# microsoft/EVA

Hardware: AMD Instinct MI355X
Metric: homomorphic ops/sec (mul+rescale+relin) at N=2^16, L=10; execute() wall-time (higher is better)
Workload: dtype u64

## Files before the change

eva_amd/csrc/internal.hip.h:

```cpp
#pragma once
#include "../../include/eva_hip.h"

#include <hip/hip_runtime.h>

#include <algorithm>
#include <cmath>
#include <cstdlib>
#include <cstring>
#include <functional>
#include <map>
#include <memory>
#include <mutex>
#include <stdexcept>
#include <string>
#include <tuple>
#include <unordered_map>
#include <vector>

#include "devmath.hip.h"
#include "hostmath.h"

namespace evah {

extern thread_local std::string g_err;

void ctx_register(const void *c);
void ctx_unregister(const void *c);
bool ctx_alive(const void *c);

#define HIPCHK(x)                                                                                \
  do {                                                                                           \
    hipError_t e_ = (x);                                                                         \
    if (e_ != hipSuccess)                                                                        \
      throw std::runtime_error(std::string(#x) + " failed: " + hipGetErrorString(e_));          \
  } while (0)

#ifndef EVAH_KS_BATCH_MAX_DEFINED
#define EVAH_KS_BATCH_MAX_DEFINED
constexpr int KS_BATCH_MAX = 64;
#endif


struct Pool {
  std::map<size_t, std::vector<void *>> free_;
  size_t in_use = 0, cached = 0;
  void *alloc(size_t bytes) {
    bytes = (bytes + 255) & ~(size_t)255;
    auto it = free_.find(bytes);
    void *p = nullptr;
    if (it != free_.end() && !it->second.empty()) {
      p = it->second.back();
      it->second.pop_back();
      cached -= bytes;
    } else {
      hipError_t e = hipMalloc(&p, bytes);
      if (e != hipSuccess) {
        release_cached();
        HIPCHK(hipMalloc(&p, bytes));
      }
    }
    in_use += bytes;
    return p;
  }
  void free(void *p, size_t bytes) {
    bytes = (bytes + 255) & ~(size_t)255;
    free_[bytes].push_back(p);
    in_use -= bytes;
    cached += bytes;
  }
  void release_cached() {
    for (auto &kv : free_)
      for (void *p : kv.second) (void)hipFree(p);
    free_.clear();
    cached = 0;
  }
};

struct Buffer {
  u64 *d;
  size_t bytes;
  int refs;
  Pool *pool;
  evah_ctx *owner;
  bool ready_everywhere;
  std::vector<evah_ctx *> synced;
  std::vector<evah_ctx *> readers;
};

enum KClass {
  KC_EW = 0,
  KC_INTT_A,
  KC_INTT_B,
  KC_KSDIGIT_A,
  KC_KSDIGIT_B,
  KC_KSMAC,
  KC_MODDOWN_A,
  KC_MODDOWN_B,
  KC_NTT_A,
  KC_NTT_B,
  KC_COUNT
};
static const char *const kclass_names[KC_COUNT] = {
    "elementwise", "intt_pass1", "intt_pass2", "ksdigit_pass1", "ksdigit_pass2", "ks_mac",
    "moddown_pass1", "moddown_pass2", "ntt_pass1", "ntt_pass2"};

struct ProfRec {
  hipEvent_t e0, e1;
  int cls;
};

__host__ __device__ inline size_t keyp_block_words(uint32_t nd) { return ((size_t)2 * nd + 1) * 256; }
struct KeyDev {
  u64 *d = nullptr;
  uint32_t n_digits = 0;
  size_t bytes = 0;
  uint32_t rows = 0;
  u64 *d_split = nullptr;
  u64 *d_perm = nullptr;
};

}

using namespace evah;

struct evah_ct {
  Buffer *buf;
  u64 *d;
  uint32_t size, limbs;
  size_t ps;
  double scale;
  uint32_t batch = 1;
};
struct evah_pt {
  Buffer *buf;
  u64 *d;
  uint32_t limbs;
  double scale;
  bool uniform = false;
};
struct evah_graph {
  hipGraph_t graph = nullptr;
  hipGraphExec_t exec = nullptr;
  struct Reserved { evah_ctx *ctx; void *p; size_t bytes; };
  std::vector<Reserved> reserved;
};

struct SharedDev {
  int device = 0;
  void *d_tables = nullptr;
  KeyDev relin;
  KeyDev pk, sk;
  double2 *dec_roots = nullptr;
  std::map<uint32_t, u64 *> crt_tabs;
  std::map<uint32_t, KeyDev> galois;
  std::map<uint32_t, uint32_t *> perms;
  std::map<uint32_t, uint32_t *> perms_inv;
  std::map<uint32_t, u64 *> hoist_sign;
  std::map<std::pair<uint32_t, uint32_t>, u64 *> hoist_corr;
  double2 *enc_roots = nullptr;
  double enc_last_root[2] = {0, 0};
  uint32_t *enc_slot_map = nullptr;
  uint32_t key_rows = 0, key_shard = 0;
  uint64_t xfer[6] = {0, 0, 0, 0, 0, 0};
  uint64_t key_up[2] = {0, 0};
  ~SharedDev() {
    (void)hipSetDevice(device);
    if (enc_roots) (void)hipFree(enc_roots);
    if (enc_slot_map) (void)hipFree(enc_slot_map);
    if (relin.d) (void)hipFree(relin.d);
    if (relin.d_split) (void)hipFree(relin.d_split);
    if (pk.d) (void)hipFree(pk.d);
    if (sk.d) { (void)hipMemset(sk.d, 0, sk.bytes); (void)hipFree(sk.d); }
    if (dec_roots) (void)hipFree(dec_roots);
    for (auto &kv : crt_tabs) (void)hipFree(kv.second);
    for (auto &kv : galois) {
      (void)hipFree(kv.second.d);
      if (kv.second.d_split) (void)hipFree(kv.second.d_split);
      if (kv.second.d_perm) (void)hipFree(kv.second.d_perm);
    }
    for (auto &kv : perms) (void)hipFree(kv.second);
    for (auto &kv : perms_inv) (void)hipFree(kv.second);
    for (auto &kv : hoist_sign) (void)hipFree(kv.second);
    for (auto &kv : hoist_corr) (void)hipFree(kv.second);
    if (d_tables) (void)hipFree(d_tables);
  }
};

struct Tunables {
  bool fuse_mac = true;
  bool fuse_mul = true;
  bool fuse_mul2 = true;
  bool ew_fuse = true;
  bool ew_uniform = true;
  uint32_t fuse_small_blocks = 2048;
  int small_lr = 2;
  uint32_t small_lr_blocks = 1024;
  bool hoist = true;
  uint32_t hoist_min_tiles = 2048;
  bool hoist_debug = false;
  bool peer_self_check = false;
  bool hoist_table_fail = false;
  bool fuse_special_inv = true;
  int ks_groups = 1;
  int ks_threads = 64;
  bool fold_pa = true;
  bool win_fuse = true;
  bool win_linear = true;
  bool fb_persist = true;
  uint32_t fb_grid = 0;
  bool mac3 = true;
  uint32_t loop_n = 8, loop_min = 2, loop_min_wgs = 2048, loop_target_wgs = 8192;
  bool hoist_map = true;
  uint32_t hoist_v = 1;
  bool side_stream = false;
  bool chain_step = true, chain_batched = true;
  uint32_t chain_fuse_blocks = 256;
  bool modup = true;
  uint32_t lds_extra = 0;

  static Tunables from_env(uint32_t N) {
    Tunables t;
    auto flag = [](const char *name, bool &v) { if (const char *e = std::getenv(name)) v = std::atoi(e) != 0; };
    auto count = [](const char *name, uint32_t &v) { if (const char *e = std::getenv(name)) v = (uint32_t)std::max(0, std::atoi(e)); };
    (void)N;
    flag("EVAH_FUSE_MAC", t.fuse_mac);
    flag("EVAH_FUSE_MUL", t.fuse_mul);
    flag("EVAH_FUSE_MUL2", t.fuse_mul2);
    flag("EVAH_EW_FUSE", t.ew_fuse);
    flag("EVAH_EW_UNIFORM", t.ew_uniform);
    count("EVAH_FUSE_SMALL", t.fuse_small_blocks);
    if (const char *e = std::getenv("EVAH_SMALL_LR")) t.small_lr = std::atoi(e) == 3 ? 3 : 2;
    count("EVAH_SMALL_LR_BLOCKS", t.small_lr_blocks);
    flag("EVAH_HOIST", t.hoist);
    count("EVAH_HOIST_MIN_TILES", t.hoist_min_tiles);
    flag("EVAH_HOIST_DEBUG", t.hoist_debug);
    flag("EVAH_HOIST_TABLE_FAIL", t.hoist_table_fail);
    flag("EVAH_PEER_SELF_CHECK", t.peer_self_check);
    flag("EVAH_FUSE_SPECIAL_INV", t.fuse_special_inv);
    flag("EVAH_FOLD_PA", t.fold_pa);
    flag("EVAH_WIN_FUSE", t.win_fuse);
    flag("EVAH_WIN_LINEAR", t.win_linear);
    flag("EVAH_FB_PERSIST", t.fb_persist);
    count("EVAH_FB_GRID", t.fb_grid);
    flag("EVAH_MAC3", t.mac3);
    count("EVAH_LOOP_N", t.loop_n);
    count("EVAH_LOOP_MIN", t.loop_min);
    count("EVAH_LOOP_MIN_WGS", t.loop_min_wgs);
    count("EVAH_LOOP_TARGET_WGS", t.loop_target_wgs);
    count("EVAH_LDS_EXTRA", t.lds_extra);
    flag("EVAH_HOIST_MAP", t.hoist_map);
    flag("EVAH_SIDE_STREAM", t.side_stream);
    flag("EVAH_CHAIN_STEP", t.chain_step);
    flag("EVAH_CHAIN_BATCHED", t.chain_batched);
    count("EVAH_CHAIN_FUSE_BLOCKS", t.chain_fuse_blocks);
    flag("EVAH_MODUP", t.modup);
    count("EVAH_HOIST_V", t.hoist_v);
    if (const char *e = std::getenv("EVAH_KS_GROUPS")) t.ks_groups = std::max(1, std::atoi(e));
    if (const char *e = std::getenv("EVAH_KS_THREADS")) {
      const int n = std::atoi(e);
      if (n == 64 || n == 128 || n == 256) t.ks_threads = n;
    }
    return t;
  }
};

struct evah_ctx {
  std::shared_ptr<SharedDev> sh;
  int device = 0;
  uint32_t N = 0, logN = 0, k = 0;
  std::vector<u64> primes;
  std::vector<int> total_bits;
  DevCtx dev{};
  hipStream_t own = nullptr, stream = nullptr;
  hipStream_t side = nullptr;
  Pool pool;
  hipEvent_t ev0 = nullptr, ev1 = nullptr;
  bool capturing = false;
  std::vector<hipEvent_t> capture_events;
  std::vector<hipEvent_t> sync_events;
  Tunables tun;
  bool all_tb = false;
  bool prof_on = false;
  std::vector<ProfRec> prof_recs;
  std::vector<hipEvent_t> prof_free;
  double prof_ms[KC_COUNT] = {0};
  uint64_t prof_n[KC_COUNT] = {0};
};

namespace evah {

inline void use(evah_ctx *c) { HIPCHK(hipSetDevice(c->device)); }
inline void count_h2d(evah_ctx *c, size_t bytes, bool plain = false) { c->sh->xfer[plain ? 2 : 0]++; c->sh->xfer[4] += bytes; }
inline void count_d2h(evah_ctx *c, size_t bytes, bool plain = false) { c->sh->xfer[plain ? 3 : 1]++; c->sh->xfer[5] += bytes; }

inline hipEvent_t prof_event(evah_ctx *c) {
  if (!c->prof_free.empty()) {
    hipEvent_t e = c->prof_free.back();
    c->prof_free.pop_back();
    return e;
  }
  hipEvent_t e;
  HIPCHK(hipEventCreate(&e));
  return e;
}
inline void prof_drain(evah_ctx *c) {
  for (auto &r : c->prof_recs) {
    float ms = 0;
    HIPCHK(hipEventSynchronize(r.e1));
    HIPCHK(hipEventElapsedTime(&ms, r.e0, r.e1));
    c->prof_ms[r.cls] += ms;
    c->prof_n[r.cls]++;
    c->prof_free.push_back(r.e0);
    c->prof_free.push_back(r.e1);
  }
  c->prof_recs.clear();
}
struct ProfScope {
  evah_ctx *c;
  int cls;
  hipEvent_t e0 = nullptr;
  ProfScope(evah_ctx *c_, int cls_) : c(c_), cls(cls_) {
    if (c->prof_on && !c->capturing) {
      if (c->prof_recs.size() >= 8192) prof_drain(c);
      e0 = prof_event(c);
      HIPCHK(hipEventRecord(e0, c->stream));
    }
  }
  ~ProfScope() {
    if (e0) {
      hipEvent_t e1 = prof_event(c);
      (void)hipEventRecord(e1, c->stream);
      c->prof_recs.push_back({e0, e1, cls});
    }
  }
};

inline Buffer *buf_new(evah_ctx *c, size_t elems) {
  Buffer *b = new Buffer;
  b->bytes = elems * sizeof(u64);
  b->d = (u64 *)c->pool.alloc(b->bytes);
  b->refs = 1;
  b->pool = &c->pool;
  b->owner = c;
  b->ready_everywhere = false;
  return b;
}
inline void h2d_now(evah_ctx *c, void *dst, const void *src, size_t bytes) {
  HIPCHK(hipMemcpyAsync(dst, src, bytes, hipMemcpyHostToDevice, c->stream));
  HIPCHK(hipStreamSynchronize(c->stream));
}
inline hipEvent_t sync_event(evah_ctx *c) {
  if (!c->capturing && !c->sync_events.empty()) {
    hipEvent_t e = c->sync_events.back();
    c->sync_events.pop_back();
    return e;
  }
  hipEvent_t e;
  HIPCHK(hipEventCreateWithFlags(&e, hipEventDisableTiming));
  return e;
}
inline void stream_wait(evah_ctx *waiter, evah_ctx *signaller) {
  if (waiter == signaller || waiter->stream == signaller->stream) return;
  if (waiter->sh.get() != signaller->sh.get()) {
    int cur = 0;
    HIPCHK(hipGetDevice(&cur));
    HIPCHK(hipSetDevice(signaller->device));
    hipEvent_t e = sync_event(signaller);
    hipError_t rc = hipEventRecord(e, signaller->stream);
    (void)hipSetDevice(waiter->device);
    if (rc == hipSuccess) rc = hipStreamWaitEvent(waiter->stream, e, 0);
    (void)hipSetDevice(cur);
    if (waiter->capturing || signaller->capturing) signaller->capture_events.push_back(e);
    else signaller->sync_events.push_back(e);
    HIPCHK(rc);
    return;
  }
  hipEvent_t e = sync_event(waiter);
  HIPCHK(hipEventRecord(e, signaller->stream));
  HIPCHK(hipStreamWaitEvent(waiter->stream, e, 0));
  if (waiter->capturing || signaller->capturing) waiter->capture_events.push_back(e);
  else waiter->sync_events.push_back(e);
}
struct SideStream {
  evah_ctx *c;
  hipStream_t main;
  bool forked = false, on_side = false;
  explicit SideStream(evah_ctx *c_) : c(c_), main(c_->stream) {}
  void link(hipStream_t from, hipStream_t to) {
    hipEvent_t e = sync_event(c);
    HIPCHK(hipEventRecord(e, from));
    HIPCHK(hipStreamWaitEvent(to, e, 0));
    if (c->capturing) c->capture_events.push_back(e);
    else c->sync_events.push_back(e);
  }
  void fork() {
    if (!c->side) HIPCHK(hipStreamCreateWithFlags(&c->side, hipStreamNonBlocking));
    link(main, c->side);
    c->stream = c->side;
    forked = on_side = true;
  }
  void back() { c->stream = main; on_side = false; }
  void join() {
    back();
    if (forked) link(c->side, main);
    forked = false;
  }
  ~SideStream() {
    c->stream = main;
    if (forked) {
      hipEvent_t e = sync_event(c);
      if (hipEventRecord(e, c->side) == hipSuccess) (void)hipStreamWaitEvent(main, e, 0);
      (c->capturing ? c->capture_events : c->sync_events).push_back(e);
    }
  }
};
inline void acquire(evah_ctx *c, Buffer *b) {
  if (!b || b->owner == c) return;
  if (!b->ready_everywhere && std::find(b->synced.begin(), b->synced.end(), c) == b->synced.end()) {
    stream_wait(c, b->owner);
    b->synced.push_back(c);
  }
  if (std::find(b->readers.begin(), b->readers.end(), c) == b->readers.end()) b->readers.push_back(c);
}
inline void buf_unref(evah_ctx *c, Buffer *b) {
  (void)c;
  if (b && --b->refs == 0) {
    if (!ctx_alive(b->owner)) {
      (void)hipFree(b->d);
      delete b;
      return;
    }
    for (evah_ctx *r : b->readers)
      if (ctx_alive(r)) stream_wait(b->owner, r);
    b->pool->free(b->d, b->bytes);
    delete b;
  }
}
inline evah_ct *ct_new(evah_ctx *c, uint32_t size, uint32_t limbs, double scale, uint32_t batch = 1) {
  evah_ct *t = new evah_ct;
  t->batch = batch;
  t->buf = buf_new(c, (size_t)batch * size * limbs * c->N);
  t->d = t->buf->d;
  t->size = size;
  t->limbs = limbs;
  t->ps = (size_t)limbs * c->N;
  t->scale = scale;
  return t;
}
inline evah_pt *pt_new(evah_ctx *c, uint32_t limbs, double scale) {
  evah_pt *t = new evah_pt;
  t->buf = buf_new(c, (size_t)limbs * c->N);
  t->d = t->buf->d;
  t->limbs = limbs;
  t->scale = scale;
  return t;
}

bool hoist_wanted(const evah_ctx *c, uint32_t l, uint32_t n, uint32_t B);

KeyDev key_shape(evah_ctx *c, uint32_t n_digits);
hipError_t key_rows_h2d(evah_ctx *c, const KeyDev &kd, const u64 *src, uint32_t blocks, uint32_t first, uint32_t step);
void key_install(evah_ctx *c, int kind, uint32_t galois_elt, const KeyDev &kd);

struct Scratch {
  evah_ctx *c;
  u64 *d;
  size_t bytes;
  Scratch(evah_ctx *c_, size_t elems) : c(c_), bytes(elems * sizeof(u64)) {
    d = (u64 *)c->pool.alloc(bytes);
  }
  ~Scratch() { c->pool.free(d, bytes); }
};

inline dim3 ew_grid(evah_ctx *c, uint32_t limbs, uint32_t polys) {
  return dim3(c->N / 512, limbs, polys);
}

inline int bitlen_of_product(const std::vector<u64> &primes, uint32_t count) {
  std::vector<u64> w{1};
  for (uint32_t i = 0; i < count; i++) {
    u64 carry = 0;
    for (auto &x : w) {
      u128 t = (u128)x * primes[i] + carry;
      x = (u64)t;
      carry = (u64)(t >> 64);
    }
    if (carry) w.push_back(carry);
  }
  int bits = (int)(w.size() - 1) * 64;
  u64 top = w.back();
  while (top) { bits++; top >>= 1; }
  return bits;
}

inline void check_scale(evah_ctx *c, double scale, uint32_t limbs) {
  if (!(scale > 0) || (int)std::log2(scale) >= c->total_bits[limbs])
    throw std::invalid_argument("scale out of bounds");
}
inline bool same_scale(double a, double b) {
  double scale_factor = std::max({std::fabs(a), std::fabs(b), 1.0});
  return std::fabs(a - b) < 2.220446049250313e-16 * scale_factor;
}

}

#define EW_LAUNCH(...) do { ProfScope ps_(c, KC_EW); hipLaunchKernelGGL(__VA_ARGS__); } while (0)
#define API_BEGIN try {
#define API_END                                                                                  \
  g_err.clear();                                                                                 \
  return 0;                                                                                      \
  }                                                                                              \
  catch (const std::exception &e) {                                                              \
    g_err = e.what();                                                                            \
    return 1;                                                                                    \
  }                                                                                              \
  catch (...) {                                                                                  \
    g_err = "unknown error";                                                                     \
    return 1;                                                                                    \
  }
```

eva_amd/csrc/launch.hip.h:

```cpp
#pragma once
#include "internal.hip.h"
#include "ntt.hip.h"

namespace evah {

#define EW_SETUP                                                                                 \
  const uint32_t p = blockIdx.z, i = blockIdx.y;                                                 \
  const size_t off = (size_t)i * cx.N + 2 * ((size_t)blockIdx.x * blockDim.x + threadIdx.x);    \
  const DevPrime pm = cx.primes[cx.prime_of(i)];                                                 \
  (void)p;                                                                                        \
  (void)pm;

__device__ __forceinline__ ulonglong2 ld2(const u64 *p) { return *reinterpret_cast<const ulonglong2 *>(p); }
__device__ __forceinline__ void st2(u64 *p, ulonglong2 v) { *reinterpret_cast<ulonglong2 *>(p) = v; }
__device__ __forceinline__ u64 split30(u64 k) { return (k & 0x3fffffffull) | ((k >> 30) << 32); }

template <class Op> struct OpClass;
template <bool Z, bool G> struct OpClass<OpPlainT<Z, G>> { static constexpr int fwd_a = KC_NTT_A, fwd_b = KC_NTT_B; };
template <> struct OpClass<OpMulIntt> { static constexpr int fwd_a = KC_NTT_A, fwd_b = KC_NTT_B; };
template <> struct OpClass<OpKsDigit> { static constexpr int fwd_a = KC_KSDIGIT_A, fwd_b = KC_KSDIGIT_B; };
template <bool G> struct OpClass<OpModDownT<G>> { static constexpr int fwd_a = KC_MODDOWN_A, fwd_b = KC_MODDOWN_B; };
template <> struct OpClass<OpMulPolyIntt> { static constexpr int fwd_a = KC_NTT_A, fwd_b = KC_NTT_B; };
template <> struct OpClass<OpModDownMul> { static constexpr int fwd_a = KC_MODDOWN_A, fwd_b = KC_MODDOWN_B; };
template <int M> struct OpClass<OpRRT<M>> { static constexpr int fwd_a = KC_MODDOWN_A, fwd_b = KC_MODDOWN_B; };
template <int M> struct OpClass<OpRRLastT<M>> { static constexpr int fwd_a = KC_MODDOWN_A, fwd_b = KC_MODDOWN_B; };
template <> struct OpClass<OpChainIntt> { static constexpr int fwd_a = KC_NTT_A, fwd_b = KC_NTT_B; };
template <> struct OpClass<OpChainT> { static constexpr int fwd_a = KC_INTT_B, fwd_b = KC_INTT_B; };
template <> struct OpClass<OpChainDigit> { static constexpr int fwd_a = KC_KSDIGIT_A, fwd_b = KC_KSDIGIT_B; };
template <> struct OpClass<OpRsMd> { static constexpr int fwd_a = KC_MODDOWN_A, fwd_b = KC_MODDOWN_B; };

template <int P, int LR, bool STRIDED, bool INVERSE, class Op>
static void launch_pass(evah_ctx *c, const typename Op::Params &prm, uint32_t jobs) {
  ProfScope ps(c, INVERSE ? (STRIDED ? KC_INTT_B : KC_INTT_A)
                          : (STRIDED ? OpClass<Op>::fwd_a : OpClass<Op>::fwd_b));
  const uint32_t max_tile = (uint32_t)NTT_THREADS << LR;
  const uint32_t tile = c->N < max_tile ? c->N : max_tile;
  const int logC = (int)ilog2(tile) - P;
  size_t lds = ((((size_t)1 << logC) * lds_sub_stride<P>() + 1) & ~(size_t)1) * sizeof(u64);
  if (STRIDED) lds += ((size_t)1 << P) * sizeof(ulonglong2);
  lds += c->tun.lds_extra;
  const uint32_t n_tiles = c->N / tile;
  const int log_tiles = (int)ilog2(n_tiles);
  dim3 grid = Op::grid(prm, jobs), block(tile >> LR);
  grid.x *= n_tiles;
  if (tile == max_tile) {
    hipLaunchKernelGGL((ntt_pass_kernel<P, LR, STRIDED, INVERSE, Op, true>), grid, block, lds, c->stream, c->dev,
                       prm, logC, log_tiles);
  } else if constexpr (P == 5) {
    hipLaunchKernelGGL((ntt_pass_kernel<P, LR, STRIDED, INVERSE, Op, false>), grid, block, lds, c->stream, c->dev,
                       prm, logC, log_tiles);
  } else {
    throw std::logic_error("partial NTT tile with P != 5");
  }
  HIPCHK(hipGetLastError());
}

template <int LR, bool STRIDED, bool INVERSE, class Op>
static void launch_pass_lr(evah_ctx *c, int P, const typename Op::Params &prm, uint32_t jobs) {
  switch (P) {
  case 5: launch_pass<5, LR, STRIDED, INVERSE, Op>(c, prm, jobs); break;
  case 6: launch_pass<6, LR, STRIDED, INVERSE, Op>(c, prm, jobs); break;
  case 7: launch_pass<7, LR, STRIDED, INVERSE, Op>(c, prm, jobs); break;
  case 8: launch_pass<8, LR, STRIDED, INVERSE, Op>(c, prm, jobs); break;
  case 9:
    if constexpr (STRIDED) { launch_pass<9, LR, STRIDED, INVERSE, Op>(c, prm, jobs); break; }
    [[fallthrough]];
  default: throw std::runtime_error("unsupported poly_modulus_degree for the NTT kernels");
  }
}
template <int P, bool INVERSE, class Op>
static bool launch_loop_pass(evah_ctx *c, const typename Op::Params &prm, uint32_t jobs) {
  constexpr int LR = 2;
  dim3 grid = Op::grid(prm, jobs);
  uint32_t ext[3] = {grid.x, grid.y, grid.z};
  const uint32_t count = ext[Op::loop_axis];
  if (!c->tun.loop_n || count < c->tun.loop_min || c->N < 256) return false;
  if ((uint64_t)ext[0] * ext[1] * ext[2] / count * (c->N / 256) * ((count + 1) / 2) < c->tun.loop_min_wgs) return false;
  ProfScope ps(c, INVERSE ? KC_INTT_A : OpClass<Op>::fwd_b);
  const uint32_t tile = 256, n_tiles = c->N / tile;
  const int logC = 8 - P, log_tiles = (int)ilog2(n_tiles);
  uint32_t nloop = std::min<uint32_t>(c->tun.loop_n, count);
  const uint64_t others = (uint64_t)ext[0] * ext[1] * ext[2] / count * n_tiles;
  while (nloop > 2 && others * ((count + nloop - 1) / nloop) < c->tun.loop_target_wgs) nloop = (nloop + 1) / 2;
  ext[Op::loop_axis] = (count + nloop - 1) / nloop;
  const size_t lds = ((((size_t)1 << logC) * lds_sub_stride<P>() + 1) & ~(size_t)1) * sizeof(u64) +
                     ((size_t)1 << (logC + P)) * sizeof(ulonglong2);
  hipLaunchKernelGGL((ntt_loop_kernel<P, LR, INVERSE, Op>), dim3(ext[0] * n_tiles, ext[1], ext[2]), dim3(tile >> LR), lds, c->stream,
                     c->dev, prm, logC, log_tiles, nloop, count);
  HIPCHK(hipGetLastError());
  return true;
}
template <bool INVERSE, class Op>
static bool launch_loop_pass_p(evah_ctx *c, int P, const typename Op::Params &prm, uint32_t jobs) {
  switch (P) {
  case 5: return launch_loop_pass<5, INVERSE, Op>(c, prm, jobs);
  case 6: return launch_loop_pass<6, INVERSE, Op>(c, prm, jobs);
  case 7: return launch_loop_pass<7, INVERSE, Op>(c, prm, jobs);
  case 8: return launch_loop_pass<8, INVERSE, Op>(c, prm, jobs);
  default: return false;
  }
}

template <bool STRIDED, bool INVERSE, class Op>
static void launch_pass_p(evah_ctx *c, int P, const typename Op::Params &prm, uint32_t jobs) {
  if constexpr (!STRIDED) {
    if (launch_loop_pass_p<INVERSE, Op>(c, P, prm, jobs)) return;
  }
  if (c->tun.small_lr == 2 && (uint64_t)jobs * (c->N >> 11) <= c->tun.small_lr_blocks && c->N >= 2048) {
    launch_pass_lr<2, STRIDED, INVERSE, Op>(c, P, prm, jobs);
    return;
  }
  launch_pass_lr<3, STRIDED, INVERSE, Op>(c, P, prm, jobs);
}

struct KsBatch {
  uint32_t n = 1;
  uint32_t i0 = 0, ni = 0;
  size_t target_bs = 0, scratch_bs = 0, prod_bs = 0;
  KsKeys keys{};
  PtrTab targets{};
  const MulTab *mul = nullptr;
  bool fold = false;
  const PtrTab *adds = nullptr;
  bool mac3 = false;
  bool lazy_out = false;
  uint32_t istep = 1, nout = 0;
  u64 *r_out = nullptr;
  bool diag = false;
  uint32_t fold_row = ~0u;
};
void launch_ks_inner(evah_ctx *c, int P, const u64 *target, const u64 *scratch, const KsBatch &key, u64 *prod, uint32_t l);

template <class Op> static void ntt_forward(evah_ctx *c, const typename Op::Params &prm, uint32_t jobs) {
  const int a = (c->logN + 1) / 2, b = c->logN / 2;
  launch_pass_p<true, false, Op>(c, a, prm, jobs);
  launch_pass_p<false, false, Op>(c, b, prm, jobs);
}
template <class Op> static void ntt_inverse(evah_ctx *c, const typename Op::Params &prm, uint32_t jobs) {
  const int a = (c->logN + 1) / 2, b = c->logN / 2;
  launch_pass_p<false, true, Op>(c, b, prm, jobs);
  launch_pass_p<true, true, Op>(c, a, prm, jobs);
}

static inline bool fuse_small_launch(evah_ctx *c, uint32_t fwd_jobs) {
  const uint32_t tile = (uint32_t)NTT_THREADS << 3;
  if (!c->tun.fuse_small_blocks || c->N < tile) return false;
  if (c->dev.guard) return true;
  return (uint64_t)fwd_jobs * (c->N / tile) <= c->tun.fuse_small_blocks;
}
template <int P, class Op, int LR> static void launch_inv_fwd_plr(evah_ctx *c, const typename Op::Params &prm, uint32_t jobs) {
  ProfScope ps(c, OpClass<Op>::fwd_a);
  const uint32_t tile = (uint32_t)NTT_THREADS << LR, n_tiles = c->N / tile;
  const int logC = (int)ilog2(tile) - P;
  const size_t lds = ((((size_t)1 << logC) * lds_sub_stride<P>() + 1) & ~(size_t)1) * sizeof(u64) + 2 * ((size_t)1 << P) * sizeof(ulonglong2);
  dim3 grid = Op::grid(prm, jobs);
  grid.x *= n_tiles;
  hipLaunchKernelGGL((ntt_inv_fwd_kernel<P, LR, Op>), grid, dim3(NTT_THREADS), lds, c->stream, c->dev, prm, (int)ilog2(n_tiles));
  HIPCHK(hipGetLastError());
}
template <int P, class Op> static void launch_inv_fwd_p(evah_ctx *c, const typename Op::Params &prm, uint32_t jobs) {
  if (c->tun.small_lr == 2) launch_inv_fwd_plr<P, Op, 2>(c, prm, jobs);
  else launch_inv_fwd_plr<P, Op, 3>(c, prm, jobs);
}
template <class Op> static void launch_inv_fwd(evah_ctx *c, const typename Op::Params &prm, uint32_t jobs) {
  switch ((c->logN + 1) / 2) {
  case 6: launch_inv_fwd_p<6, Op>(c, prm, jobs); break;
  case 7: launch_inv_fwd_p<7, Op>(c, prm, jobs); break;
  case 8: launch_inv_fwd_p<8, Op>(c, prm, jobs); break;
  case 9: launch_inv_fwd_p<9, Op>(c, prm, jobs); break;
  default: throw std::runtime_error("unsupported poly_modulus_degree for the fused inverse/forward pass");
  }
}
static inline bool modup_fits(evah_ctx *c) { return c->N >= ((uint32_t)NTT_THREADS << 3) && (c->logN + 1) / 2 <= 9; }
template <int P, class Op> static void launch_modup_p(evah_ctx *c, const typename Op::Params &prm, uint32_t n) {
  ProfScope ps(c, OpClass<Op>::fwd_a);
  constexpr int LR = 3;
  const uint32_t tile = (uint32_t)NTT_THREADS << LR, n_tiles = c->N / tile;
  const int logC = (int)ilog2(tile) - P;
  const size_t lds = ((((size_t)1 << logC) * lds_sub_stride<P>() + 1) & ~(size_t)1) * sizeof(u64) + ((size_t)1 << P) * sizeof(ulonglong2);
  hipLaunchKernelGGL((ntt_modup_kernel<P, LR, Op>), dim3(n_tiles * prm.l, 1, n), dim3(NTT_THREADS), lds, c->stream, c->dev, prm,
                     (int)ilog2(n_tiles));
  HIPCHK(hipGetLastError());
}
template <class Op> static void launch_modup(evah_ctx *c, const typename Op::Params &prm, uint32_t n) {
  if (!modup_fits(c) || prm.i0 != 0 || prm.istep != 1) throw std::logic_error("mod-up kernel outside its shapes");
  switch ((c->logN + 1) / 2) {
  case 6: launch_modup_p<6, Op>(c, prm, n); break;
  case 7: launch_modup_p<7, Op>(c, prm, n); break;
  case 8: launch_modup_p<8, Op>(c, prm, n); break;
  case 9: launch_modup_p<9, Op>(c, prm, n); break;
  default: throw std::runtime_error("unsupported poly_modulus_degree for the mod-up kernel");
  }
}
template <int P, class Op, bool FWD, int LR> static void launch_inv2_plr(evah_ctx *c, const typename Op::Params &prm, uint32_t jobs) {
  ProfScope ps(c, OpClass<Op>::fwd_a);
  const uint32_t tile = (uint32_t)NTT_THREADS << LR, n_tiles = c->N / tile;
  const int logC = (int)ilog2(tile) - P;
  const size_t lds = ((((size_t)1 << logC) * lds_sub_stride<P>() + 1) & ~(size_t)1) * sizeof(u64) + 2 * ((size_t)1 << P) * sizeof(ulonglong2);
  dim3 grid = Op::grid(prm, jobs);
  grid.x *= n_tiles;
  hipLaunchKernelGGL((ntt_inv2_kernel<P, LR, Op, FWD>), grid, dim3(NTT_THREADS), lds, c->stream, c->dev, prm, (int)ilog2(n_tiles));
  HIPCHK(hipGetLastError());
}
template <class Op, bool FWD> static void launch_inv2(evah_ctx *c, const typename Op::Params &prm, uint32_t jobs) {
  auto go = [&](auto ptag) {
    constexpr int P = decltype(ptag)::value;
    if (c->tun.small_lr == 2) launch_inv2_plr<P, Op, FWD, 2>(c, prm, jobs);
    else launch_inv2_plr<P, Op, FWD, 3>(c, prm, jobs);
  };
  switch ((c->logN + 1) / 2) {
  case 6: go(std::integral_constant<int, 6>{}); break;
  case 7: go(std::integral_constant<int, 7>{}); break;
  case 8: go(std::integral_constant<int, 8>{}); break;
  case 9: go(std::integral_constant<int, 9>{}); break;
  default: throw std::runtime_error("unsupported poly_modulus_degree for the fused inverse/forward pass");
  }
}
template <class InvOp, class Op>
static void inverse_then_forward(evah_ctx *c, const typename InvOp::Params &ip, uint32_t inv_jobs, const typename Op::Params &fp,
                                 uint32_t fwd_jobs, bool inv_pass1_done = false) {
  if (inv_pass1_done && !fuse_small_launch(c, fwd_jobs)) throw std::logic_error("fused inverse pass outside the small-launch form");
  if (fuse_small_launch(c, fwd_jobs)) {
    if (!inv_pass1_done) launch_pass_p<false, true, InvOp>(c, c->logN / 2, ip, inv_jobs);
    launch_inv_fwd<Op>(c, fp, fwd_jobs);
    launch_pass_p<false, false, Op>(c, c->logN / 2, fp, fwd_jobs);
  } else {
    ntt_inverse<InvOp>(c, ip, inv_jobs);
    ntt_forward<Op>(c, fp, fwd_jobs);
  }
}

bool switch_key_products(evah_ctx *c, uint32_t l, const u64 *target, size_t target_bs, const KeyDev *const *keys, uint32_t n,
                         u64 *prod_d, const PtrTab *target_tab = nullptr, const MulTab *mul = nullptr, u64 *r_small = nullptr,
                         bool fold = false, const PtrTab *adds = nullptr, bool lazy_out = false);
void switch_key(evah_ctx *c, uint32_t l, const u64 *target, const KeyDev &key, const u64 *add, size_t add_ps, uint32_t add_polys,
                u64 *out, size_t out_ps);
void key_split_launch(evah_ctx *c, const u64 *src, u64 *dst, size_t words);
const uint32_t *perm_table(evah_ctx *c, uint32_t elt);
void galois_perm_launch(evah_ctx *c, const u64 *a, size_t a_ps, uint32_t limbs, uint32_t polys, const uint32_t *perm, u64 *out, size_t o_ps);
void enc_tables(evah_ctx *c);

}
```

eva_amd/csrc/ntt_modup.hip.h:

```cpp
#pragma once
#include "ntt.hip.h"

namespace evah {

template <int P, int LR, class Op>
__global__ void __launch_bounds__(NTT_THREADS)
ntt_modup_kernel(DevCtx cx, typename Op::Params prm, int log_tiles) {
  extern __shared__ __attribute__((aligned(16))) u64 lds[];
  constexpr int NTT_R = 1 << LR;
  constexpr int S = 1 << P, TPS = S / NTT_R, SP = lds_sub_stride<P>();
  constexpr int logC = 8 + LR - P, C = 1 << logC, T = NTT_THREADS;
  constexpr int TWR = (S + T - 1) / T;
  if (cx.skipped()) return;
  const uint32_t tile_idx = blockIdx.x & ((1u << log_tiles) - 1u), J = blockIdx.x >> log_tiles, b = blockIdx.z;
  typename Op::Job jb;
  uint32_t iy = 0;
  while (iy < prm.ni && !Op::setup(cx, prm, J, iy, b, jb)) iy++;
  if (iy >= prm.ni) return;
  const uint32_t pa = Op::pre_prime(prm, jb);
  const DevPrime pmA = cx.primes[pa];
  const uint32_t stride_log = cx.logN - P;
  constexpr int ES = 1 << (P - LR);
  constexpr bool LINEAR = (ES % 16 == 0);
  const int c = threadIdx.x & (C - 1), e0 = threadIdx.x >> logC;
  const uint32_t n0 = (tile_idx << logC) + ((uint32_t)e0 << stride_log) + c, nstep = (uint32_t)(T >> logC) << stride_log;
  const int l0 = c * SP + lds_pad<P>(e0);
  auto lds_at = [&](int it) -> int {
    if constexpr (LINEAR) return l0 + it * lds_pad<P>(ES);
    const int idx = threadIdx.x + it * T;
    return (idx & (C - 1)) * SP + lds_pad<P>(idx >> logC);
  };
  const u64 *src = Op::pre_src(jb);
#pragma unroll
  for (int it = 0; it < NTT_R; it++) lds[lds_at(it)] = src[n0 + it * nstep];
  ulonglong2 *twl = reinterpret_cast<ulonglong2 *>(lds + ((C * SP + 1) & ~1));
  const ulonglong2 *twA = cx.tw_inv + (size_t)pa * cx.N;
  for (int idx = threadIdx.x; idx < S; idx += T) twl[idx] = twA[idx];
  ulonglong2 twn[TWR];
  auto tw_request = [&](uint32_t prime) {
    const ulonglong2 *tw = cx.tw_fwd + (size_t)prime * cx.N;
#pragma unroll
    for (int r = 0; r < TWR; r++)
      if (S >= T || (int)threadIdx.x + r * T < S) twn[r] = tw[threadIdx.x + r * T];
  };
  tw_request(jb.prime);
  __syncthreads();
  const int sub = threadIdx.x / TPS, tid = threadIdx.x % TPS;
  RoundSeq<P, LR, 0, true, true, false>::run(lds + sub * SP, tid, 0, 0, twl, pmA);
  __syncthreads();
  u64 t[NTT_R];
#pragma unroll
  for (int it = 0; it < NTT_R; it++) {
    t[it] = lds[lds_at(it)];
    if (Op::pre_addhalf) t[it] = addmod(t[it], pmA.q >> 1, pmA.q);
  }
  while (true) {
#pragma unroll
    for (int r = 0; r < TWR; r++)
      if (S >= T || (int)threadIdx.x + r * T < S) twl[threadIdx.x + r * T] = twn[r];
    const DevPrime pm = cx.primes[jb.prime];
    auto convert = [&](auto lazy_tag) {
      constexpr bool LZ = decltype(lazy_tag)::value;
#pragma unroll
      for (int it = 0; it < NTT_R; it++) lds[lds_at(it)] = Op::template conv<LZ>(jb, pm, t[it]);
    };
    if (jb.lazy) convert(std::true_type{});
    else convert(std::false_type{});
    typename Op::Job jn;
    uint32_t in = iy + 1;
    while (in < prm.ni && !Op::setup(cx, prm, J, in, b, jn)) in++;
    const bool more = in < prm.ni;
    if (more) tw_request(jn.prime);
    __syncthreads();
    forward_rounds<P, LR, true, false>(lds + sub * SP, tid, 0, 0, twl, pm);
    __syncthreads();
#pragma unroll
    for (int it = 0; it < NTT_R; it++) jb.dst[n0 + it * nstep] = lds[lds_at(it)];
    if (!more) break;
    jb = jn;
    iy = in;
  }
}

}
```

Before: 15590.

## Keep mod-up NTT data in registers across rounds with double-buffered twiddles

Adds a register-resident variant of the fused inverse-NTT/base-conversion/forward-NTT mod-up kernel. The inverse result stays in registers, and each output prime's conversion and first forward round start straight from registers instead of a full LDS write and read-back. It also uses a new column-padded LDS layout and double-buffers the forward twiddles so staging the next prime overlaps the current one. The variant is on by default behind a tunable; it needs more LDS for the second twiddle buffer and more registers, which may lower occupancy.

```diff
diff --git a/eva_amd/csrc/internal.hip.h b/eva_amd/csrc/internal.hip.h
--- a/eva_amd/csrc/internal.hip.h
+++ b/eva_amd/csrc/internal.hip.h
@@ -216,6 +216,7 @@
   bool chain_step = true, chain_batched = true;
   uint32_t chain_fuse_blocks = 256;
   bool modup = true;
+  bool modup_regs = true;
   uint32_t lds_extra = 0;
 
   static Tunables from_env(uint32_t N) {
@@ -254,6 +255,7 @@
     flag("EVAH_CHAIN_BATCHED", t.chain_batched);
     count("EVAH_CHAIN_FUSE_BLOCKS", t.chain_fuse_blocks);
     flag("EVAH_MODUP", t.modup);
+    flag("EVAH_MODUP_REGS", t.modup_regs);
     count("EVAH_HOIST_V", t.hoist_v);
     if (const char *e = std::getenv("EVAH_KS_GROUPS")) t.ks_groups = std::max(1, std::atoi(e));
     if (const char *e = std::getenv("EVAH_KS_THREADS")) {
diff --git a/eva_amd/csrc/launch.hip.h b/eva_amd/csrc/launch.hip.h
--- a/eva_amd/csrc/launch.hip.h
+++ b/eva_amd/csrc/launch.hip.h
@@ -176,10 +176,14 @@
   ProfScope ps(c, OpClass<Op>::fwd_a);
   constexpr int LR = 3;
   const uint32_t tile = (uint32_t)NTT_THREADS << LR, n_tiles = c->N / tile;
-  const int logC = (int)ilog2(tile) - P;
-  const size_t lds = ((((size_t)1 << logC) * lds_sub_stride<P>() + 1) & ~(size_t)1) * sizeof(u64) + ((size_t)1 << P) * sizeof(ulonglong2);
-  hipLaunchKernelGGL((ntt_modup_kernel<P, LR, Op>), dim3(n_tiles * prm.l, 1, n), dim3(NTT_THREADS), lds, c->stream, c->dev, prm,
-                     (int)ilog2(n_tiles));
+  const dim3 grid(n_tiles * prm.l, 1, n);
+  constexpr size_t lds_regs = modup_lds_bytes<P, LR, true>(), lds_tile = modup_lds_bytes<P, LR, false>();
+  if (c->tun.modup_regs)
+    hipLaunchKernelGGL((ntt_modup_kernel<P, LR, Op, true>), grid, dim3(NTT_THREADS), lds_regs, c->stream, c->dev, prm,
+                       (int)ilog2(n_tiles));
+  else
+    hipLaunchKernelGGL((ntt_modup_kernel<P, LR, Op, false>), grid, dim3(NTT_THREADS), lds_tile, c->stream, c->dev, prm,
+                       (int)ilog2(n_tiles));
   HIPCHK(hipGetLastError());
 }
 template <class Op> static void launch_modup(evah_ctx *c, const typename Op::Params &prm, uint32_t n) {
diff --git a/eva_amd/csrc/ntt_modup.hip.h b/eva_amd/csrc/ntt_modup.hip.h
--- a/eva_amd/csrc/ntt_modup.hip.h
+++ b/eva_amd/csrc/ntt_modup.hip.h
@@ -3,7 +3,202 @@
 
 namespace evah {
 
+template <int P> struct ModupTile {
+  static constexpr int SH = P == 6 ? 4 : P == 8 ? 2 : 3;
+  static constexpr int SP = P == 6 ? 69 : P == 7 ? 143 : P == 8 ? 322 : 580;
+  static __device__ __forceinline__ int pad(int e) { return e + (e >> SH); }
+  static_assert(SP >= (1 << P) + (((1 << P) - 1) >> SH), "a column holds every padded element");
+};
+template <int P, int LR, int RB, int LO> struct ColRound {
+  static constexpr int NTT_R = 1 << LR, TPS = (1 << P) >> LR, G = NTT_R >> RB, NU = 1 << RB;
+  static constexpr int S0 = P - LO - RB;
+  using L = ModupTile<P>;
+  static __device__ __forceinline__ int o_hi(int g, int p) { return (g * TPS + p) >> LO; }
+  static __device__ __forceinline__ int ebase(int g, int p) {
+    const int o = g * TPS + p;
+    return ((o >> LO) << (LO + RB)) | (o & ((1 << LO) - 1));
+  }
+  static __device__ __forceinline__ void load(const u64 *col, int p, u64 (&x)[NTT_R]) {
+#pragma unroll
+    for (int g = 0; g < G; g++) {
+      const u64 *grp = col + L::pad(ebase(g, p));
+#pragma unroll
+      for (int u = 0; u < NU; u++) x[g * NU + u] = grp[L::pad(u << LO)];
+    }
+  }
+  static __device__ __forceinline__ void store(u64 *col, int p, const u64 (&x)[NTT_R]) {
+#pragma unroll
+    for (int g = 0; g < G; g++) {
+      u64 *grp = col + L::pad(ebase(g, p));
+#pragma unroll
+      for (int u = 0; u < NU; u++) grp[L::pad(u << LO)] = x[g * NU + u];
+    }
+  }
+  template <bool TB> static __device__ __forceinline__ void fwd(int p, u64 (&x)[NTT_R], const ulonglong2 *tw, const DevPrime &pm) {
+    const u64 nq = pm.nq, q4 = pm.q4, q8 = pm.q8, nq8 = pm.nq8;
+    constexpr bool MAD = EVAH_MADLO && LR == 3;
+#pragma unroll
+    for (int g = 0; g < G; g++) {
+      const uint32_t node = (1u << S0) | (uint32_t)o_hi(g, p);
+#pragma unroll
+      for (int s = 0; s < RB; s++) {
+        const int half = 1 << (RB - 1 - s);
+#pragma unroll
+        for (int u = 0; u < NU; u++) {
+          if (u & half) continue;
+          const int v = u >> (RB - s);
+          const ulonglong2 w = tw[(node << s) + v];
+          const bool red = TB ? tb_reduce_stage<P, false>(S0 + s) : (((S0 + s) & 1) != 0);
+          if (red) bfly_fwd<true, MAD, TB>(x[g * NU + u], x[g * NU + u + half], w, nq, q4, q8, nq8, pm.tb_c, pm.tb_sh, pm.tb_mask);
+          else bfly_fwd<false, MAD, TB>(x[g * NU + u], x[g * NU + u + half], w, nq, q4, q8, nq8, pm.tb_c, pm.tb_sh, pm.tb_mask);
+        }
+      }
+    }
+  }
+  static __device__ __forceinline__ void inv(int p, u64 (&x)[NTT_R], const ulonglong2 *tw, const DevPrime &pm) {
+    const u64 q = pm.q, nq = pm.nq, q5 = pm.q5, nq5 = pm.nq5;
+#pragma unroll
+    for (int g = 0; g < G; g++) {
+      const uint32_t node = (1u << S0) | (uint32_t)o_hi(g, p);
+#pragma unroll
+      for (int s = RB - 1; s >= 0; s--) {
+        const int half = 1 << (RB - 1 - s);
+        const bool last = (S0 == 0) && (s == 0);
+#pragma unroll
+        for (int u = 0; u < NU; u++) {
+          if (u & half) continue;
+          u64 &X = x[g * NU + u], &Y = x[g * NU + u + half];
+          if (last) {
+            u64 sum = X + Y, d = X + q5 - Y;
+            X = mul_shoup(sum, pm.ninv, pm.ninv_s, q);
+            Y = mul_shoup(d, pm.w0ninv, pm.w0ninv_s, q);
+          } else {
+            const int v = u >> (RB - s);
+            bfly_inv(X, Y, tw[((size_t)node << s) + v], nq, q5, nq5);
+          }
+        }
+      }
+    }
+  }
+};
+template <int P, int LR, int I, bool TB> struct ColFwd {
+  using RS = Rounds<P, LR>;
+  using R = ColRound<P, LR, RS::bits(I), RS::lo(I)>;
+  static __device__ __forceinline__ void run(u64 *col, int p_in, u64 (&x)[1 << LR], const ulonglong2 *tw, const DevPrime &pm) {
+    int p = p_in;
+    if constexpr (I > 0) R::load(col, p, x);
+    else if constexpr (TB) asm volatile("" : "+v"(p));
+    R::template fwd<TB>(p, x, tw, pm);
+    if constexpr (I + 1 < RS::NR) {
+      R::store(col, p, x);
+      __syncthreads();
+      ColFwd<P, LR, I + 1, TB>::run(col, p, x, tw, pm);
+    }
+  }
+};
+template <int P, int LR, int I> struct ColInv {
+  using RS = Rounds<P, LR>;
+  static constexpr int idx = RS::NR - 1 - I;
+  using R = ColRound<P, LR, RS::bits(idx), RS::lo(idx)>;
+  static __device__ __forceinline__ void run(u64 *col, int p, u64 (&x)[1 << LR], const ulonglong2 *tw, const DevPrime &pm) {
+    R::load(col, p, x);
+    R::inv(p, x, tw, pm);
+    if constexpr (idx > 0) {
+      R::store(col, p, x);
+      __syncthreads();
+      ColInv<P, LR, I + 1>::run(col, p, x, tw, pm);
+    }
+  }
+};
+template <int P, int LR, bool REGS> constexpr size_t modup_lds_bytes() {
+  constexpr size_t C = (size_t)1 << (8 + LR - P), S = (size_t)1 << P;
+  if (REGS) return ((C * ModupTile<P>::SP + 1) & ~(size_t)1) * sizeof(u64) + 2 * S * sizeof(ulonglong2);
+  return ((C * lds_sub_stride<P>() + 1) & ~(size_t)1) * sizeof(u64) + S * sizeof(ulonglong2);
+}
+
 template <int P, int LR, class Op>
+__device__ __forceinline__ void modup_regs(const DevCtx &cx, const typename Op::Params &prm, int log_tiles, u64 *lds) {
+  constexpr int NTT_R = 1 << LR;
+  constexpr int S = 1 << P, TPS = S / NTT_R;
+  constexpr int logC = 8 + LR - P, C = 1 << logC, T = NTT_THREADS;
+  constexpr int TWR = (S + T - 1) / T;
+  using L = ModupTile<P>;
+  using RS = Rounds<P, LR>;
+  using RLast = ColRound<P, LR, RS::bits(RS::NR - 1), 0>;
+  static_assert(RS::bits(0) == LR && RS::lo(0) == P - LR && RS::lo(RS::NR - 1) == 0, "round 0 works on the load mapping's elements");
+  const uint32_t tile_idx = blockIdx.x & ((1u << log_tiles) - 1u), J = blockIdx.x >> log_tiles, b = blockIdx.z;
+  typename Op::Job jb;
+  uint32_t iy = 0;
+  while (iy < prm.ni && !Op::setup(cx, prm, J, iy, b, jb)) iy++;
+  if (iy >= prm.ni) return;
+  const uint32_t pa = Op::pre_prime(prm, jb);
+  const DevPrime pmA = cx.primes[pa];
+  const uint32_t stride_log = cx.logN - P;
+  const int c = threadIdx.x & (C - 1), p = threadIdx.x >> logC;
+  const uint32_t gcol = (tile_idx << logC) + c;
+  const uint32_t nlast = gcol + ((uint32_t)(p * RLast::NU) << stride_log);
+  u64 *col = lds + c * L::SP;
+  const u64 *src = Op::pre_src(jb);
+#pragma unroll
+  for (int u = 0; u < NTT_R; u++) col[L::pad(p) + L::pad(u * TPS)] = (src + ((size_t)(u * TPS) << stride_log))[gcol + ((uint32_t)p << stride_log)];
+  ulonglong2 *twl = reinterpret_cast<ulonglong2 *>(lds + ((C * L::SP + 1) & ~1));
+  const ulonglong2 *twA = cx.tw_inv + (size_t)pa * cx.N;
+  for (int idx = threadIdx.x; idx < S; idx += T) twl[idx] = twA[idx];
+  ulonglong2 twn[TWR];
+  auto tw_request = [&](uint32_t prime) {
+    const ulonglong2 *tw = cx.tw_fwd + (size_t)prime * cx.N;
+#pragma unroll
+    for (int r = 0; r < TWR; r++)
+      if (S >= T || (int)threadIdx.x + r * T < S) twn[r] = tw[threadIdx.x + r * T];
+  };
+  auto tw_stage = [&](int buf) {
+#pragma unroll
+    for (int r = 0; r < TWR; r++)
+      if (S >= T || (int)threadIdx.x + r * T < S) twl[buf * S + threadIdx.x + r * T] = twn[r];
+  };
+  tw_request(jb.prime);
+  tw_stage(1);
+  __syncthreads();
+  u64 t[NTT_R];
+  ColInv<P, LR, 0>::run(col, p, t, twl, pmA);
+  if (Op::pre_addhalf) {
+#pragma unroll
+    for (int u = 0; u < NTT_R; u++) t[u] = addmod(t[u], pmA.q >> 1, pmA.q);
+  }
+  int cur = 1;
+  while (true) {
+    const DevPrime pm = cx.primes[jb.prime];
+    typename Op::Job jn;
+    uint32_t in = iy + 1;
+    while (in < prm.ni && !Op::setup(cx, prm, J, in, b, jn)) in++;
+    const bool more = in < prm.ni;
+    if (more) tw_request(jn.prime);
+    u64 x[NTT_R];
+    if (jb.lazy) {
+#pragma unroll
+      for (int u = 0; u < NTT_R; u++) x[u] = Op::template conv<true>(jb, pm, t[u]);
+    } else {
+#pragma unroll
+      for (int u = 0; u < NTT_R; u++) x[u] = Op::template conv<false>(jb, pm, t[u]);
+    }
+    const ulonglong2 *tw = twl + cur * S;
+    if (EVAH_TOPBIT && pm.tb_c) ColFwd<P, LR, 0, true>::run(col, p, x, tw, pm);
+    else ColFwd<P, LR, 0, false>::run(col, p, x, tw, pm);
+#pragma unroll
+    for (int g = 0; g < RLast::G; g++)
+#pragma unroll
+      for (int u = 0; u < RLast::NU; u++)
+        (jb.dst + ((size_t)(g * TPS * RLast::NU + u) << stride_log))[nlast] = x[g * RLast::NU + u];
+    if (!more) break;
+    tw_stage(cur ^ 1);
+    __syncthreads();
+    jb = jn;
+    iy = in;
+    cur ^= 1;
+  }
+}
+
+template <int P, int LR, class Op, bool REGS = false>
 __global__ void __launch_bounds__(NTT_THREADS)
 ntt_modup_kernel(DevCtx cx, typename Op::Params prm, int log_tiles) {
   extern __shared__ __attribute__((aligned(16))) u64 lds[];
@@ -12,6 +207,10 @@
   constexpr int logC = 8 + LR - P, C = 1 << logC, T = NTT_THREADS;
   constexpr int TWR = (S + T - 1) / T;
   if (cx.skipped()) return;
+  if constexpr (REGS) {
+    modup_regs<P, LR, Op>(cx, prm, log_tiles, lds);
+    return;
+  }
   const uint32_t tile_idx = blockIdx.x & ((1u << log_tiles) - 1u), J = blockIdx.x >> log_tiles, b = blockIdx.z;
   typename Op::Job jb;
   uint32_t iy = 0;
```

New measurement: 15710, median of 5. About the same (+0.7%).
